# arcee-ai/DALM

Measured on NVIDIA H100. Metric: RAG-e2e train-step samples/sec (bge-large + Llama-2-7B, bs=18), higher is better.
Workload: dtype bf16

## Files before the change

### dalm_b200/_lib.py

```python
from __future__ import annotations

import ctypes
import os
from ctypes import c_char_p, c_float, c_int, c_longlong, c_void_p

_HERE = os.path.dirname(os.path.abspath(__file__))
LIB_PATH = os.path.join(_HERE, "csrc", "libdalm_b200.so")

from ctypes import c_ulonglong

_I, _L, _F, _P, _U = c_int, c_longlong, c_float, c_void_p, c_ulonglong
_DROP = [_F, _U, _U, _P]

SIGNATURES = {
    "dalm_b200_last_error": [],
    "dalm_b200_version": [],
    "dalm_b200_launch_count": [],
    "dalm_b200_reset_launch_count": [],
    "dalm_b200_probe_device": [],
    "dalm_b200_marginal_counts": [_P, _P, _I, _I, _P, _P, _P],
    "dalm_b200_inbatch_loss_fwd_bwd": [_P, _P, _I, _I, _F, _P, _P, _P, _P, _P, _P, _P, _F, _P],
    "dalm_b200_ce_marginal_fwd_bwd": [_P, _P, _I, _P, _P, _P, _P, _I, _I, _I, _L, _F, _P],
    "dalm_b200_ce_marginal_rows": [_P, _P, _I, _P, _P, _P, _P, _I, _I, _I, _L, _F, _I, _I, _P],
    "dalm_b200_finalize_loss": [_P, _P, _I, _I, _P, _P, _P, _P],
    "dalm_b200_bump_counter": [_P, _P],
    "dalm_b200_dropout_scale": [_P, _L, _F, _U, _U, _P, _P],
    "dalm_b200_lora_dx": [_P, _L, _P, _L, _P, _L, _I, _I, _I, _F, _U, _U, _P, _P],
    "dalm_b200_small_matmul_f32": [_P, _P, _P, _I, _I, _I, _I, _I, _F, _P],
    "dalm_b200_gemm_bf16": [_I, _P, _L, _P, _L, _P, _L, _I, _I, _I, _I, _F, _P, _I, _P, _L, _I, _I, _I, *_DROP, _P],
    "dalm_b200_gemm_clear_cache": [],
    "dalm_b200_gemm_set_raster": [_I],
    "dalm_b200_gemm_set_l2_hints": [_I],
    "dalm_b200_attention_fwd": [_P, _L, _P, _L, _P, _L, _P, _P, _L, _P, _I, _I, _I, _I, _I, _F, _I, _I, *_DROP, _P],
    "dalm_b200_attention_tc_fwd": [_P, _L, _P, _L, _P, _L, _P, _P, _L, _P, _I, _I, _I, _I, _I, _F, _I, _I, *_DROP, _P],
    "dalm_b200_attention_tc_bwd": [_P, _L, _P, _L, _P, _L, _P, _P, _L, _P, _P, _L, _P, _P, _L, _P, _L, _P, _L,
                                   _I, _I, _I, _I, _I, _F, _I, _I, *_DROP, _P],
    "dalm_b200_attention_bwd": [_P, _L, _P, _L, _P, _L, _P, _P, _L, _P, _P, _L, _P, _P, _L, _P, _L, _P, _L,
                                _I, _I, _I, _I, _I, _F, _I, _I, *_DROP, _P],
    "dalm_b200_layernorm_fwd": [_P, _P, _P, _P, _P, _L, _P, _P, _I, _I, _F, *_DROP, _P],
    "dalm_b200_layernorm_bwd": [_P, _P, _P, _P, _P, _P, _L, _P, _P, _L, _I, _I, *_DROP, _P],
    "dalm_b200_layernorm_bwd_res": [_P, _P, _P, _P, _P, _P, _L, _P, _P, _P, _L, _I, _I, _P],
    "dalm_b200_rmsnorm_fwd": [_P, _P, _P, _L, _P, _I, _I, _F, _P],
    "dalm_b200_rmsnorm_bwd": [_P, _P, _P, _P, _L, _P, _P, _P, _L, _I, _I, _P],
    "dalm_b200_bert_embed": [_P, _P, _P, _P, _P, _I, _I, _I, _I, _P],
    "dalm_b200_roberta_embed": [_P, _P, _P, _P, _I, _P, _P, _I, _I, _I, _I, _I, _P],
    "dalm_b200_embed_gather": [_P, _P, _P, _I, _I, _I, _P],
    "dalm_b200_rope": [_P, _L, _I, _I, _I, _P, _P, _I, _I, _I, _P],
# ... 40 lines not shown
    "dalm_b200_moe_router_bwd": [_P, _L, _P, _P, _P, _I, _I, _I, _I, _P, _L, _P],
    "dalm_b200_moe_permute": [_P, _I, _I, _I, _P, _P, _P, _P, _P, _P, _P, _P],
    "dalm_b200_moe_gather": [_P, _L, _I, _I, _P, _I, _P, _I, _P, _L, _P],
    "dalm_b200_moe_combine": [_P, _L, _P, _P, _I, _I, _I, _P, _L, _P, _L, _I, _P],
    "dalm_b200_moe_down_bwd": [_P, _L, _P, _L, _P, _P, _I, _I, _P, _P, _L, _P],
}
_RESTYPES = {
    "dalm_b200_last_error": c_char_p,
    "dalm_b200_version": c_char_p,
    "dalm_b200_launch_count": c_longlong,
    "dalm_b200_topk_ip_workspace": c_longlong,
    "dalm_b200_reset_launch_count": None,
    "dalm_b200_gemm_clear_cache": None,
    "dalm_b200_gemm_set_raster": None,
    "dalm_b200_gemm_set_l2_hints": None,
}

_lib = None


class DalmB200Error(RuntimeError):
    pass


def load() -> ctypes.CDLL:
    global _lib
    if _lib is not None:
        return _lib
    if not os.path.exists(LIB_PATH):
        raise DalmB200Error(
# ... 31 lines not shown
```

### dalm_b200/csrc/gemm_wgmma.cu

```cuda
#include "common.cuh"
#include "ptx.cuh"
#include <cudaTypedefs.h>
#include <mutex>
#include <unordered_map>

namespace dalm {
using namespace ptx;

enum class Epi {
  Plain,
  SwiGLU,
  RoPE,
  GeluPair,
  NormRoPE,
};

struct GemmEpilogue {
  void* out;
  long long ldo;
  int out_f32;
  const float* bias;
  const void* resid;
  long long ldr;
  int resid_f32;
// ... 17 lines not shown
__device__ __forceinline__ void tile_coords(int tile, int num_m, int num_n, int gm, int& m_blk, int& n_blk) {
  if (gm <= 0) { m_blk = tile % num_m; n_blk = tile / num_m; return; }
  const int band_tiles = gm * num_n;
  const int band = tile / band_tiles;
  const int r = tile - band * band_tiles;
  const int m0 = band * gm;
  const int h = min(gm, num_m - m0);
  const int n = r / h;
  m_blk = m0 + (r - n * h);
  n_blk = (band & 1) ? (num_n - 1 - n) : n;
}

constexpr int kBoxRows = 64;
constexpr int kBoxBytes = kBoxRows * 128;
constexpr int kStageTileBytes = 2 * kBoxBytes;
constexpr int kEpiGroups = 2;
constexpr int kGemmThreads = 128 + kEpiGroups * 128;

struct EpiStage {
  unsigned char* boxes;
  int bar;
  bool issuer;
  int buf;
  __device__ __forceinline__ unsigned char* begin() {
    if (issuer) bulk_wait_read<1>();
    named_bar_sync(bar, 128);
    return boxes + buf * kBoxBytes;
  }
  __device__ __forceinline__ void end(const CUtensorMap* tm, int col, int row, bool evict_first) {
    fence_proxy_async();
    named_bar_sync(bar, 128);
    if (issuer) {
// ... 267 lines not shown
    }
    sg.end(tmap_out, col0, row0, hint);
    if constexpr (EPI == Epi::GeluPair) {
      box = sg.begin();
#pragma unroll
      for (int i = 0; i < 16; ++i) {
        const float2 p = __bfloat1622float2(pk[i]);
        box_st_bf16x2(box, rb + 8 * (i & 1), 16 * (i >> 1) + 4 * k, gelu_erf(p.x), gelu_erf(p.y));
      }
      sg.end(tmap_out2, col0, row0, false);
    }
    shift8();
  }
}

template <int BN> struct GemmCfg {
  static constexpr int BM = 128, BK = 64;
  static constexpr int A_BYTES = BM * BK * 2;
  static constexpr int B_BYTES = BN * BK * 2;
  static constexpr int STAGE_BYTES = A_BYTES + B_BYTES;
  static constexpr int STAGES = (BN == 256) ? 4 : (BN == 128 ? 6 : 8);
  static constexpr int SMEM_BYTES = STAGES * STAGE_BYTES + kEpiGroups * kStageTileBytes + 1024  + 256 ;
  static_assert(SMEM_BYTES <= 232448, "exceeds 227 KB of shared memory per block");
};

template <int BN, int TA, int TB>
__device__ __forceinline__ void wgmma_tile(float* d, uint64_t da, uint64_t db, int scale_d) {
  if constexpr (BN == 256) wgmma_m64n256k16<TA, TB>(d, da, db, scale_d);
  else if constexpr (BN == 128) wgmma_m64n128k16<TA, TB>(d, da, db, scale_d);
  else wgmma_m64n64k16<TA, TB>(d, da, db, scale_d);
}

template <int BN, int LAYOUT, Epi EPI, int CL, bool GROUPED>
__global__ void __launch_bounds__(kGemmThreads, 1)
gemm_bf16_tn_kernel(const __grid_constant__ CUtensorMap tmap_a, const __grid_constant__ CUtensorMap tmap_b,
                    const __grid_constant__ CUtensorMap tmap_out, const __grid_constant__ CUtensorMap tmap_out2, const GemmEpilogue ep) {
  using Cfg = GemmCfg<BN>;
  constexpr int BM = Cfg::BM, BK = Cfg::BK, STAGES = Cfg::STAGES;
  static_assert(CL == 1 || (LAYOUT == 0 && EPI == Epi::Plain), "the cluster kernel takes the plain TN layout");
  static_assert(!GROUPED || (CL == 1 && LAYOUT <= 1), "the grouped kernel takes the TN and NN layouts on single CTAs");
  extern __shared__ unsigned char smem_raw[];
  unsigned char* smem = reinterpret_cast<unsigned char*>((reinterpret_cast<uintptr_t>(smem_raw) + 1023) & ~uintptr_t(1023));
  unsigned char* staging = smem + STAGES * Cfg::STAGE_BYTES;
  uint64_t* full_bar  = reinterpret_cast<uint64_t*>(staging + kEpiGroups * kStageTileBytes);
  uint64_t* empty_bar = full_bar + STAGES;

  const int warp = threadIdx.x >> 5, lane = threadIdx.x & 31;
  const uint32_t rank = CL == 2 ? cluster_ctarank() : 0u;
  const int M = ep.M, N = ep.N, K = ep.K;
  const int num_m = GROUPED ? min((M + BM - 1) / BM, __ldg(ep.grp_live)) : (M + CL * BM - 1) / (CL * BM);
  const int num_n = (N + BN - 1) / BN;
  const int num_tiles = num_m * num_n;
  const int num_kb = (K + BK - 1) / BK;
  const int unit = blockIdx.x / CL, num_units = gridDim.x / CL;
  const int group_m = CL == 2 ? 0 : ep.group_m;

  if (threadIdx.x == 0) {
    prefetch_tmap(&tmap_a);
    prefetch_tmap(&tmap_b);
    prefetch_tmap(&tmap_out);
    if constexpr (EPI == Epi::SwiGLU || EPI == Epi::GeluPair || EPI == Epi::NormRoPE) prefetch_tmap(&tmap_out2);
  }
  if (threadIdx.x == 32) {
    for (int s = 0; s < STAGES; ++s) { mbar_init(&full_bar[s], 1); mbar_init(&empty_bar[s], 8 * CL); }
    fence_mbar_init();
  }
  if constexpr (CL == 2) cluster_sync_all();
  else __syncthreads();

  if (warp < 4) {
    asm volatile("setmaxnreg.dec.sync.aligned.u32 40;" ::: "memory");
    if (warp == 0 && lane == 0) {
      int stage = 0; uint32_t phase = 0;
      const bool hint_a = (ep.l2_hints & 1) != 0, hint_b = (ep.l2_hints & 2) != 0;
      const uint64_t pol_a = hint_a ? l2_policy_evict_last() : 0ull, pol_b = hint_b ? l2_policy_evict_first() : 0ull;
      auto load = [](void* dst, const CUtensorMap* tm, uint64_t* bar, int c0, int c1, bool hinted, uint64_t pol) {
        if (hinted) tma_load_2d_hint(dst, tm, bar, c0, c1, pol);
        else        tma_load_2d(dst, tm, bar, c0, c1);
      };
      for (int tile = unit; tile < num_tiles; tile += num_units) {
        int m_blk, n_blk;
        tile_coords(tile, num_m, num_n, group_m, m_blk, n_blk);
        const int b_row0 = GROUPED ? __ldg(ep.grp_tiles + m_blk) * (LAYOUT == 1 ? K : N) : 0;
        for (int kb = 0; kb < num_kb; ++kb) {
          mbar_wait(&empty_bar[stage], phase ^ 1);
          unsigned char* sa = smem + stage * Cfg::STAGE_BYTES;
// ... 9 lines not shown
            } else {
              load(sa, &tmap_a, &full_bar[stage], kb * BK, m_blk * BM, hint_a, pol_a);
            }
            if constexpr (LAYOUT >= 1) {
#pragma unroll
              for (int c = 0; c < BN / 64; ++c) load(sb + c * 8192, &tmap_b, &full_bar[stage], n_blk * BN + c * 64, b_row0 + kb * BK, hint_b, pol_b);
            } else {
              load(sb, &tmap_b, &full_bar[stage], kb * BK, b_row0 + n_blk * BN, hint_b, pol_b);
            }
          }
          if (++stage == STAGES) { stage = 0; phase ^= 1; }
        }
      }
    }
  } else {
    asm volatile("setmaxnreg.inc.sync.aligned.u32 232;" ::: "memory");
    const int grp = (warp - 4) >> 2;
    EpiStage sg{staging + grp * kStageTileBytes, 1 + grp, (threadIdx.x & 127) == 0, 0};
    constexpr int TA = LAYOUT == 2 ? 1 : 0, TB = LAYOUT >= 1 ? 1 : 0;
    constexpr uint64_t a_step = TA ? 128 : 2, b_step = TB ? 128 : 2;
    const uint32_t a_off = (uint32_t)grp * 8192u;
    int stage = 0; uint32_t phase = 0;
    for (int tile = unit; tile < num_tiles; tile += num_units) {
      int m_blk, n_blk;
      tile_coords(tile, num_m, num_n, group_m, m_blk, n_blk);
      float acc[BN / 2];
      int prev = -1;
      for (int kb = 0; kb < num_kb; ++kb) {
        mbar_wait(&full_bar[stage], phase);
        const uint32_t sa = smem_u32(smem + stage * Cfg::STAGE_BYTES);
        const uint32_t sb = sa + Cfg::A_BYTES;
        const uint64_t adesc = TA ? make_sw128_mnmajor_desc(sa + a_off, 8192, 1024) : make_sw128_kmajor_desc(sa + a_off);
        const uint64_t bdesc = TB ? make_sw128_mnmajor_desc(sb, 8192, 1024) : make_sw128_kmajor_desc(sb);
        wgmma_fence();
#pragma unroll
        for (int k = 0; k < BK / 16; ++k)
          wgmma_tile<BN, TA, TB>(acc, adesc + a_step * (uint64_t)k, bdesc + b_step * (uint64_t)k, (kb | k) != 0 ? 1 : 0);
        wgmma_commit();
        wgmma_wait<1>();
        if (prev >= 0 && lane == 0) {
          mbar_arrive(&empty_bar[prev]);
          if constexpr (CL == 2) mbar_arrive_remote(&empty_bar[prev], rank ^ 1u);
        }
        prev = stage;
        if (++stage == STAGES) { stage = 0; phase ^= 1; }
      }
      wgmma_wait<0>();
      if (lane == 0) {
        mbar_arrive(&empty_bar[prev]);
        if constexpr (CL == 2) mbar_arrive_remote(&empty_bar[prev], rank ^ 1u);
      }
      epilogue_tile<BN, EPI>(ep, &tmap_out, &tmap_out2, sg, acc, (m_blk * CL + (int)rank) * BM + grp * 64, n_blk * BN);
// ... 51 lines not shown
  CUtensorMap m;
  CUresult r = fn(&m, f32 ? CU_TENSOR_MAP_DATA_TYPE_FLOAT32 : CU_TENSOR_MAP_DATA_TYPE_BFLOAT16, 2, const_cast<void*>(ptr), dims, strides, box, estr,
                  CU_TENSOR_MAP_INTERLEAVE_NONE, CU_TENSOR_MAP_SWIZZLE_128B, CU_TENSOR_MAP_L2_PROMOTION_L2_256B,
                  CU_TENSOR_MAP_FLOAT_OOB_FILL_NONE);
  DALM_REQUIRE(r == CUDA_SUCCESS, "gemm: cuTensorMapEncodeTiled failed (%d) rows=%lld cols=%lld ld=%lld box_rows=%d",
               (int)r, rows, cols, ld, box_rows);
  {
    std::lock_guard<std::mutex> g(g_tmap_mu);
    if (g_tmaps.size() > 8192) g_tmaps.clear();
    g_tmaps[key] = m;
  }
  *out = m;
  return 0;
}

template <int BN, int LAYOUT, Epi EPI, bool GROUPED = false>
static int launch_gemm(const CUtensorMap& ta, const CUtensorMap& tb, const CUtensorMap& to, const GemmEpilogue& ep,
                       int max_ctas, cudaStream_t stream, const CUtensorMap* to2) {
  using Cfg = GemmCfg<BN>;
  static bool attr_set = false;
  if (!attr_set) {
    DALM_CUDA(cudaFuncSetAttribute(gemm_bf16_tn_kernel<BN, LAYOUT, EPI, 1, GROUPED>, cudaFuncAttributeMaxDynamicSharedMemorySize, Cfg::SMEM_BYTES));
    attr_set = true;
  }
  const int num_tiles = ((ep.M + 127) / 128) * ((ep.N + BN - 1) / BN);
  int grid = num_tiles < num_sms() ? num_tiles : num_sms();
  if (max_ctas > 0 && grid > max_ctas) grid = max_ctas;
  gemm_bf16_tn_kernel<BN, LAYOUT, EPI, 1, GROUPED><<<grid, kGemmThreads, Cfg::SMEM_BYTES, stream>>>(ta, tb, to, to2 ? *to2 : to, ep);
  count_launch();
  return check_launch("gemm_bf16_tn_kernel");
}

template <int LAYOUT, Epi EPI, bool GROUPED = false>
static int launch_gemm_bn(int bn, const CUtensorMap& ta, const CUtensorMap& tb, const CUtensorMap& to, const GemmEpilogue& ep,
                          int max_ctas, cudaStream_t stream, const CUtensorMap* to2 = nullptr) {
  if (bn == 256) return launch_gemm<256, LAYOUT, EPI, GROUPED>(ta, tb, to, ep, max_ctas, stream, to2);
  if (bn == 128) return launch_gemm<128, LAYOUT, EPI, GROUPED>(ta, tb, to, ep, max_ctas, stream, to2);
  return launch_gemm<64, LAYOUT, EPI, GROUPED>(ta, tb, to, ep, max_ctas, stream, to2);
}

template <int BN>
static int launch_gemm_cluster(const CUtensorMap& ta, const CUtensorMap& tb, const CUtensorMap& to, const GemmEpilogue& ep,
                               int max_ctas, cudaStream_t stream) {
  using Cfg = GemmCfg<BN>;
  auto kern = gemm_bf16_tn_kernel<BN, 0, Epi::Plain, 2, false>;
  static bool attr_set = false;
  if (!attr_set) {
    DALM_CUDA(cudaFuncSetAttribute(kern, cudaFuncAttributeMaxDynamicSharedMemorySize, Cfg::SMEM_BYTES));
    attr_set = true;
  }
  const int num_tiles = ((ep.M + 255) / 256) * ((ep.N + BN - 1) / BN);
  int clusters = num_tiles < num_sms() / 2 ? num_tiles : num_sms() / 2;
  if (max_ctas > 0 && clusters > max_ctas / 2) clusters = max_ctas / 2 > 0 ? max_ctas / 2 : 1;
  cudaLaunchConfig_t cfg = {};
  cfg.gridDim = dim3(2 * clusters);
  cfg.blockDim = dim3(kGemmThreads);
  cfg.dynamicSmemBytes = Cfg::SMEM_BYTES;
  cfg.stream = stream;
  cudaLaunchAttribute attr[1];
  attr[0].id = cudaLaunchAttributeClusterDimension;
  attr[0].val.clusterDim.x = 2; attr[0].val.clusterDim.y = 1; attr[0].val.clusterDim.z = 1;
  cfg.attrs = attr; cfg.numAttrs = 1;
  DALM_CUDA(cudaLaunchKernelEx(&cfg, kern, ta, tb, to, to, ep));
  count_launch();
  return check_launch("gemm_bf16_tn_kernel (cluster of 2)");
}

}

using namespace dalm;

static int env_int(const char* name, int dflt) {
  const char* v = getenv(name);
  return (v && *v) ? atoi(v) : dflt;
}
static int g_group_m_override = env_int("DALM_B200_GEMM_RASTER", 0);
extern "C" void dalm_b200_gemm_set_raster(int group_m) { g_group_m_override = group_m; }
static int g_l2_hints = env_int("DALM_B200_GEMM_L2_HINTS", -1);
static double l2_resident_a() { return (double)l2_bytes() / 3.0; }
extern "C" void dalm_b200_gemm_set_l2_hints(int mask) { g_l2_hints = mask < 0 ? -1 : (mask & 7); }
static int pick_l2_hints(int M, int N, int K, int tile_n, int group_m, bool stream_out) {
  if (g_l2_hints >= 0) return g_l2_hints;
  const long long tiles = (long long)((M + 127) / 128) * ((N + tile_n - 1) / tile_n);
  return (group_m == 0 && tiles > num_sms() && 2.0 * M * K <= l2_resident_a() && !stream_out) ? 7 : 0;
}

static int pick_block_n(int M, int N) {
  const long long m1 = (M + 127) / 128;
  double best = 1e30;
  int bn = 64;
  const int cand[3] = {256, 128, 64};
  const double penalty[3] = {1.0, 1.55, 2.7};
  for (int i = 0; i < 3; ++i) {
    if (cand[i] > 64 && N < cand[i]) continue;
    const long long tiles = m1 * ((N + cand[i] - 1) / cand[i]);
    const double cost = (double)((tiles + num_sms() - 1) / num_sms()) * cand[i] * penalty[i];
    if (cost < best) { best = cost; bn = cand[i]; }
  }
  return bn;
}

static int pick_group_m(int M, int N, int K, int tile_n, bool stream_out) {
  const int num_m = (M + 127) / 128, num_n = (N + tile_n - 1) / tile_n;
  int group_m = 0;
  if (g_group_m_override > 0) return g_group_m_override;
  if (g_group_m_override == -1 || (long long)num_m * num_n <= num_sms()) return 0;
  const double a_bytes = 2.0 * M * K;
  if (g_group_m_override == 0 && a_bytes <= l2_resident_a() && !stream_out) return 0;
  const double ideal = sqrt((double)num_sms() * tile_n / 128.0);
  int nbands = (int)(num_m / ideal + 0.5);
  if (nbands < 1) nbands = 1;
  group_m = (num_m + nbands - 1) / nbands;
  if (group_m >= num_m) group_m = 0;
  return group_m;
}

static GemmEpilogue gemm_epilogue(int M, int N, int K, int tile_n, void* out, long long ldo, int out_f32 = 0,
                                  const void* resid = nullptr, long long ldr = 0, int resid_f32 = 0) {
  GemmEpilogue ep{};
  ep.out = out; ep.ldo = ldo; ep.out_f32 = out_f32;
  ep.resid = resid; ep.ldr = ldr; ep.resid_f32 = resid_f32;
  ep.alpha = 1.f;
  ep.M = M; ep.N = N; ep.K = K;
  ep.drop = make_drop(0.f, 0, 0, nullptr);
  const bool stream_out = out_f32 != 0 || resid != nullptr;
  ep.group_m = pick_group_m(M, N, K, tile_n, stream_out);
  ep.l2_hints = pick_l2_hints(M, N, K, tile_n, ep.group_m, stream_out);
  return ep;
}

extern "C" int dalm_b200_gemm_bf16(int layout, const void* A, long long lda, const void* B, long long ldb, void* out,
                                   long long ldo, int out_f32, int M, int N, int K, float alpha, const float* bias,
                                   int act, const void* resid, long long ldr, int resid_f32, int block_n,
                                   int max_ctas, float drop_p, unsigned long long drop_seed,
                                   unsigned long long drop_stream_id, const void* drop_offset, void* stream) {
  DALM_REQUIRE(layout >= 0 && layout <= 2, "gemm: layout must be 0 (TN), 1 (NN) or 2 (wgrad)");
  DALM_REQUIRE(M > 0 && N > 0 && K > 0, "gemm: empty problem M=%d N=%d K=%d", M, N, K);
  DALM_REQUIRE((N % 8) == 0, "gemm: N=%d must be a multiple of 8", N);
  DALM_REQUIRE((K % 8) == 0 || layout == 2, "gemm: K=%d must be a multiple of 8", K);
  DALM_REQUIRE((M % 8) == 0 || layout != 2, "gemm: M=%d must be a multiple of 8 for the wgrad layout", M);
  DALM_REQUIRE(lda >= (layout == 2 ? M : K) && ldb >= (layout >= 1 ? N : K) && ldo >= N, "gemm: leading dimensions too small");
  DALM_REQUIRE((ldo % (out_f32 ? 4 : 8)) == 0, "gemm: ldo=%lld breaks 16-byte row alignment", ldo);
  DALM_REQUIRE((reinterpret_cast<uintptr_t>(out) & 15) == 0, "gemm: out is not 16-byte aligned");
  if (resid) {
    DALM_REQUIRE((ldr % (resid_f32 ? 4 : 8)) == 0, "gemm: ldr=%lld breaks 16-byte row alignment", ldr);
    DALM_REQUIRE((reinterpret_cast<uintptr_t>(resid) & 15) == 0, "gemm: resid is not 16-byte aligned");
  }
  DALM_REQUIRE(act == 0 || act == 1 || act == 2, "gemm: act must be 0 (none), 1 (gelu) or 2 (gelu backward: multiply by gelu'(resid))");
  DALM_REQUIRE(act != 2 || (resid != nullptr && !resid_f32 && !out_f32 && drop_p == 0.f),
               "gemm: act 2 (gelu backward) needs a bf16 `resid` (the pre-activation), a bf16 output and no dropout");
  int bn = block_n;
  if (bn == 0) bn = pick_block_n(M, N);
  DALM_REQUIRE(bn == 64 || bn == 128 || bn == 256 || bn == 2128 || bn == 2256,
               "gemm: block_n must be 0, 64/128/256 (single CTA) or 2128/2256 (cluster of two CTAs)");
  const bool pair = bn > 1000;
  DALM_REQUIRE(!(pair && layout != 0), "gemm: the cluster kernel only takes the TN layout");
  const int tile_n = pair ? bn % 1000 : bn;
  CUtensorMap ta, tb, to;
  if (layout == 2) { if (int e = get_tmap(A, K, M, lda, 64, &ta)) return e; }
  else             { if (int e = get_tmap(A, M, K, lda, 128, &ta)) return e; }
  if (layout >= 1) { if (int e = get_tmap(B, K, N, ldb, 64, &tb)) return e; }
  else             { if (int e = get_tmap(B, N, K, ldb, pair ? tile_n / 2 : tile_n, &tb)) return e; }
  if (int e = get_tmap(out, M, N, ldo, kBoxRows, &to, out_f32)) return e;
  DALM_REQUIRE(drop_p >= 0.f && drop_p < 1.f, "gemm: dropout p must be in [0,1)");
  GemmEpilogue ep = gemm_epilogue(M, N, K, tile_n, out, ldo, out_f32, resid, ldr, resid_f32);
  ep.bias = bias; ep.act = act; ep.alpha = alpha;
  ep.drop = make_drop(drop_p, drop_seed, drop_stream_id, drop_offset);
  cudaStream_t st = (cudaStream_t)stream;
  if (bn == 2256) return launch_gemm_cluster<256>(ta, tb, to, ep, max_ctas, st);
  if (bn == 2128) return launch_gemm_cluster<128>(ta, tb, to, ep, max_ctas, st);
  if (layout == 1) return launch_gemm_bn<1, Epi::Plain>(bn, ta, tb, to, ep, max_ctas, st);
  if (layout == 2) return launch_gemm_bn<2, Epi::Plain>(bn, ta, tb, to, ep, max_ctas, st);
  return launch_gemm_bn<0, Epi::Plain>(bn, ta, tb, to, ep, max_ctas, st);
}

extern "C" int dalm_b200_gemm_bf16_swiglu(const void* A, long long lda, const void* B, long long ldb, void* gu, long long ldgu,
                                          void* act, long long ldact, int M, int N, int K, void* stream) {
  DALM_REQUIRE(M > 0 && K > 0 && N >= 256 && (N % 256) == 0, "gemm_swiglu: N=%d must be a positive multiple of 256 (128-feature gate / up blocks)", N);
  DALM_REQUIRE((K % 8) == 0 && lda >= K && ldb >= K && ldgu >= N && ldact >= N / 2, "gemm_swiglu: bad K / leading dimensions");
  DALM_REQUIRE((ldgu % 8) == 0 && (ldact % 8) == 0 && ((uintptr_t)gu & 15) == 0 && ((uintptr_t)act & 15) == 0, "gemm_swiglu: output alignment");
  CUtensorMap ta, tb, to, to2;
  if (int e = get_tmap(A, M, K, lda, 128, &ta)) return e;
  if (int e = get_tmap(B, N, K, ldb, 256, &tb)) return e;
  if (int e = get_tmap(gu, M, N, ldgu, kBoxRows, &to, 0)) return e;
  if (int e = get_tmap(act, M, N / 2, ldact, kBoxRows, &to2, 0)) return e;
  const GemmEpilogue ep = gemm_epilogue(M, N, K, 256, gu, ldgu);
  return launch_gemm<256, 0, Epi::SwiGLU>(ta, tb, to, ep, 0, (cudaStream_t)stream, &to2);
}

extern "C" int dalm_b200_gemm_bf16_gelu(const void* A, long long lda, const void* B, long long ldb, void* pre, long long ldpre,
                                        void* act, long long ldact, int M, int N, int K, const float* bias, void* stream) {
  DALM_REQUIRE(M > 0 && N > 0 && K > 0 && (N % 8) == 0 && (K % 8) == 0, "gemm_gelu: bad shape M=%d N=%d K=%d", M, N, K);
  DALM_REQUIRE(lda >= K && ldb >= K && ldpre >= N && ldact >= N, "gemm_gelu: leading dimensions too small");
  DALM_REQUIRE((ldpre % 8) == 0 && (ldact % 8) == 0 && ((uintptr_t)pre & 15) == 0 && ((uintptr_t)act & 15) == 0, "gemm_gelu: output alignment");
  const int bn = pick_block_n(M, N);
  CUtensorMap ta, tb, to, to2;
  if (int e = get_tmap(A, M, K, lda, 128, &ta)) return e;
  if (int e = get_tmap(B, N, K, ldb, bn, &tb)) return e;
  if (int e = get_tmap(pre, M, N, ldpre, kBoxRows, &to, 0)) return e;
  if (int e = get_tmap(act, M, N, ldact, kBoxRows, &to2, 0)) return e;
  GemmEpilogue ep = gemm_epilogue(M, N, K, bn, pre, ldpre);
  ep.bias = bias;
  return launch_gemm_bn<0, Epi::GeluPair>(bn, ta, tb, to, ep, 0, (cudaStream_t)stream, &to2);
}

extern "C" int dalm_b200_gemm_bf16_rope(const void* A, long long lda, const void* B, long long ldb, void* out, long long ldo, int M,
                                        int N, int K, const float* bias, const float* cos_t, const float* sin_t, int L, int rope_cols,
                                        const float* q_norm, const float* k_norm, int nq_heads, float eps, void* pre_out,
                                        long long ld_pre, float* rstd_out, long long ld_rstd, void* stream) {
  DALM_REQUIRE(M > 0 && N > 0 && K > 0 && (N % 8) == 0 && (K % 8) == 0, "gemm_rope: bad shape M=%d N=%d K=%d", M, N, K);
  DALM_REQUIRE(rope_cols > 0 && rope_cols <= N && (rope_cols % 256) == 0, "gemm_rope: rope_cols=%d must be a multiple of 256 (whole 128-wide heads per tile)", rope_cols);
  DALM_REQUIRE(L > 0 && cos_t != nullptr && sin_t != nullptr && ((uintptr_t)cos_t & 15) == 0 && ((uintptr_t)sin_t & 15) == 0, "gemm_rope: cos / sin tables");
  DALM_REQUIRE(lda >= K && ldb >= K && ldo >= N && (ldo % 8) == 0 && ((uintptr_t)out & 15) == 0, "gemm_rope: leading dimensions / alignment");
  CUtensorMap ta, tb, to;
  if (int e = get_tmap(A, M, K, lda, 128, &ta)) return e;
  if (int e = get_tmap(B, N, K, ldb, 256, &tb)) return e;
  if (int e = get_tmap(out, M, N, ldo, kBoxRows, &to, 0)) return e;
  GemmEpilogue ep = gemm_epilogue(M, N, K, 256, out, ldo);
  ep.bias = bias;
  ep.rope_cos = cos_t; ep.rope_sin = sin_t; ep.rope_L = L; ep.rope_cols = rope_cols;
  if (q_norm == nullptr) {
    DALM_REQUIRE(k_norm == nullptr && pre_out == nullptr && rstd_out == nullptr, "gemm_rope: k_norm / pre_out / rstd_out need q_norm");
    return launch_gemm<256, 0, Epi::RoPE>(ta, tb, to, ep, 0, (cudaStream_t)stream, nullptr);
  }
  DALM_REQUIRE(k_norm != nullptr && nq_heads >= 0 && nq_heads <= rope_cols / 128 && eps >= 0.f, "gemm_rope: norm weights / nq_heads=%d", nq_heads);
  DALM_REQUIRE(rstd_out == nullptr || ld_rstd >= rope_cols / 128, "gemm_rope: ld_rstd=%lld < %d heads", ld_rstd, rope_cols / 128);
  CUtensorMap to2 = to;
  if (pre_out != nullptr) {
    DALM_REQUIRE(ld_pre >= rope_cols && (ld_pre % 8) == 0 && ((uintptr_t)pre_out & 15) == 0, "gemm_rope: pre_out leading dimension / alignment");
    if (int e = get_tmap(pre_out, M, rope_cols, ld_pre, kBoxRows, &to2, 0)) return e;
  }
  ep.q_norm = q_norm; ep.k_norm = k_norm; ep.nq_heads = nq_heads; ep.norm_eps = eps;
  ep.norm_rstd = rstd_out; ep.ld_rstd = ld_rstd; ep.norm_pre = pre_out != nullptr;
  return launch_gemm<256, 0, Epi::NormRoPE>(ta, tb, to, ep, 0, (cudaStream_t)stream, &to2);
}

extern "C" int dalm_b200_gemm_bf16_grouped(int layout, int swiglu, const void* A, long long lda, const void* B, int E, void* out,
                                           long long ldo, void* out2, long long ldo2, int M, int N, int K, const int* tile_expert,
                                           const int* live_tiles, int max_ctas, void* stream) {
  DALM_REQUIRE(layout == 0 || layout == 1, "gemm_grouped: layout must be 0 (TN) or 1 (NN)");
  DALM_REQUIRE(M > 0 && N > 0 && K > 0 && E > 0 && (N % 8) == 0 && (K % 8) == 0, "gemm_grouped: bad shape M=%d N=%d K=%d E=%d", M, N, K, E);
  DALM_REQUIRE(layout == 0 || (K % 64) == 0, "gemm_grouped: the NN layout needs K=%d to be a multiple of 64", K);
  DALM_REQUIRE(!swiglu || (layout == 0 && (N % 256) == 0 && out2 != nullptr && ldo2 >= N / 2 && (ldo2 % 8) == 0 &&
                           ((uintptr_t)out2 & 15) == 0),
               "gemm_grouped: swiglu needs layout 0, N=%d a multiple of 256 and an aligned out2 [M, N/2]", N);
  DALM_REQUIRE(lda >= K && ldo >= N && (ldo % 8) == 0 && ((uintptr_t)out & 15) == 0, "gemm_grouped: leading dimensions / alignment");
  DALM_REQUIRE(tile_expert != nullptr && live_tiles != nullptr, "gemm_grouped: tile_expert and live_tiles are required");
  const int bn = swiglu ? 256 : pick_block_n(M, N);
  CUtensorMap ta, tb, to, to2;
  if (int e = get_tmap(A, M, K, lda, 128, &ta)) return e;
  if (layout == 1) { if (int e = get_tmap(B, (long long)E * K, N, N, 64, &tb)) return e; }
  else             { if (int e = get_tmap(B, (long long)E * N, K, K, bn, &tb)) return e; }
  if (int e = get_tmap(out, M, N, ldo, kBoxRows, &to, 0)) return e;
  GemmEpilogue ep = gemm_epilogue(M, N, K, bn, out, ldo);
  ep.grp_tiles = tile_expert; ep.grp_live = live_tiles;
  cudaStream_t st = (cudaStream_t)stream;
  if (swiglu) {
    if (int e = get_tmap(out2, M, N / 2, ldo2, kBoxRows, &to2, 0)) return e;
    return launch_gemm<256, 0, Epi::SwiGLU, true>(ta, tb, to, ep, max_ctas, st, &to2);
  }
  if (layout == 1) return launch_gemm_bn<1, Epi::Plain, true>(bn, ta, tb, to, ep, max_ctas, st);
  return launch_gemm_bn<0, Epi::Plain, true>(bn, ta, tb, to, ep, max_ctas, st);
}

extern "C" void dalm_b200_gemm_clear_cache() {
  std::lock_guard<std::mutex> g(g_tmap_mu);
  g_tmaps.clear();
}
```

### include/dalm_b200.h

```cpp
#ifndef DALM_B200_H
#define DALM_B200_H
#include <stdint.h>
#ifdef __cplusplus
extern "C" {
#endif

const char* dalm_b200_last_error(void);
const char* dalm_b200_version(void);
long long   dalm_b200_launch_count(void);
void        dalm_b200_reset_launch_count(void);
int         dalm_b200_probe_device(void);

int dalm_b200_marginal_counts(const int64_t* gen_mask, const int64_t* qlen, int B, int L, float* cvec, float* nsum,
                              void* stream);
int dalm_b200_inbatch_loss_fwd_bwd(const float* Q, const float* P, int B, int D, float logit_scale, const float* cvec,
                                   const float* nsum, float* S, float* dlp, float* losses, float* dQ, float* dP,
                                   float grad_out, void* stream);
int dalm_b200_ce_marginal_fwd_bwd(const void* logits, void* dlogits, int dtype, const int64_t* ids, const int64_t* mask,
                                  const float* nsum, float* tok_lp, int B, int L, int V, long long ld, float grad_out,
                                  void* stream);
int dalm_b200_ce_marginal_rows(const void* logits, void* dlogits, int dtype, const int64_t* ids, const int64_t* mask,
                               const float* nsum, float* tok_lp, int B, int L, int V, long long ld, float grad_out,
                               int row0, int nrows, void* stream);
int dalm_b200_finalize_loss(const float* tok_lp, const int64_t* mask, int B, int L, const float* nsum,
// ... 12 lines not shown
int dalm_b200_gemm_bf16(int layout, const void* A, long long lda, const void* B, long long ldb, void* out, long long ldo,
                        int out_f32, int M, int N, int K, float alpha, const float* bias, int act, const void* resid,
                        long long ldr, int resid_f32, int block_n, int max_ctas, float drop_p, unsigned long long drop_seed,
                        unsigned long long drop_stream_id, const void* drop_offset, void* stream);
int dalm_b200_gemm_bf16_swiglu(const void* A, long long lda, const void* B, long long ldb, void* gu, long long ldgu, void* act,
                               long long ldact, int M, int N, int K, void* stream);
int dalm_b200_gemm_bf16_rope(const void* A, long long lda, const void* B, long long ldb, void* out, long long ldo, int M, int N,
                             int K, const float* bias, const float* cos_t, const float* sin_t, int L, int rope_cols,
                             const float* q_norm, const float* k_norm, int nq_heads, float eps, void* pre_out, long long ld_pre,
                             float* rstd_out, long long ld_rstd, void* stream);
int dalm_b200_gemm_bf16_gelu(const void* A, long long lda, const void* B, long long ldb, void* pre, long long ldpre, void* act,
                             long long ldact, int M, int N, int K, const float* bias, void* stream);
void dalm_b200_gemm_clear_cache(void);
void dalm_b200_gemm_set_raster(int group_m);
void dalm_b200_gemm_set_l2_hints(int mask);

int dalm_b200_attention_fwd(const void* q, long long ldq, const void* k, long long ldk, const void* v, long long ldv,
                            const int64_t* mask, void* out, long long ldo, float* lse, int B, int L, int Hq, int Hkv,
                            int D, float scale, int causal, int window, float drop_p, unsigned long long drop_seed,
    unsigned long long drop_stream_id, const void* drop_offset, void* stream);
int dalm_b200_attention_bwd(const void* q, long long ldq, const void* k, long long ldk, const void* v, long long ldv,
                            const int64_t* mask, const void* out, long long ldo, const float* lse, const void* d_out,
                            long long lddo, float* delta, void* dq, long long lddq, void* dk, long long lddk, void* dv,
                            long long lddv, int B, int L, int Hq, int Hkv, int D, float scale, int causal, int window, float drop_p, unsigned long long drop_seed,
    unsigned long long drop_stream_id, const void* drop_offset, void* stream);

int dalm_b200_attention_tc_fwd(const void* q, long long ldq, const void* k, long long ldk, const void* v, long long ldv,
                               const int64_t* mask, void* out, long long ldo, float* lse, int B, int L, int Hq, int Hkv,
                               int D, float scale, int causal, int window, float drop_p, unsigned long long drop_seed,
                               unsigned long long drop_stream_id, const void* drop_offset, void* stream);
// ... 127 lines not shown
```

Before: 74.01.

## Add 192x256 GEMM tiles with three consumer warpgroups for plain TN/NN GEMMs

Adds a 192-row by 256-column tile variant of the warp-specialized wgmma GEMM. It uses three epilogue/consumer warpgroups with rebalanced setmaxnreg budgets, and the stage count is now derived from the shared-memory budget. The tile picker considers the taller tile for plain TN/NN GEMMs through a wave-quantization cost model, controlled by an env flag that defaults to on. The aim is more reuse of each B tile and better wave fill. The trade-offs are fewer pipeline stages and a tighter 160-register limit for consumers, which may cause spills with the split n128 wgmma pair.

```diff
diff --git a/dalm_b200/_lib.py b/dalm_b200/_lib.py
--- a/dalm_b200/_lib.py
+++ b/dalm_b200/_lib.py
@@ -31,6 +31,7 @@
     "dalm_b200_gemm_clear_cache": [],
     "dalm_b200_gemm_set_raster": [_I],
     "dalm_b200_gemm_set_l2_hints": [_I],
+    "dalm_b200_gemm_set_tall_tiles": [_I],
     "dalm_b200_attention_fwd": [_P, _L, _P, _L, _P, _L, _P, _P, _L, _P, _I, _I, _I, _I, _I, _F, _I, _I, *_DROP, _P],
     "dalm_b200_attention_tc_fwd": [_P, _L, _P, _L, _P, _L, _P, _P, _L, _P, _I, _I, _I, _I, _I, _F, _I, _I, *_DROP, _P],
     "dalm_b200_attention_tc_bwd": [_P, _L, _P, _L, _P, _L, _P, _P, _L, _P, _P, _L, _P, _P, _L, _P, _L, _P, _L,
@@ -101,6 +102,7 @@
     "dalm_b200_gemm_clear_cache": None,
     "dalm_b200_gemm_set_raster": None,
     "dalm_b200_gemm_set_l2_hints": None,
+    "dalm_b200_gemm_set_tall_tiles": None,
 }
 
 _lib = None
diff --git a/dalm_b200/csrc/gemm_wgmma.cu b/dalm_b200/csrc/gemm_wgmma.cu
--- a/dalm_b200/csrc/gemm_wgmma.cu
+++ b/dalm_b200/csrc/gemm_wgmma.cu
@@ -55,8 +55,6 @@
 constexpr int kBoxRows = 64;
 constexpr int kBoxBytes = kBoxRows * 128;
 constexpr int kStageTileBytes = 2 * kBoxBytes;
-constexpr int kEpiGroups = 2;
-constexpr int kGemmThreads = 128 + kEpiGroups * 128;
 
 struct EpiStage {
   unsigned char* boxes;
@@ -354,35 +352,46 @@
   }
 }
 
-template <int BN> struct GemmCfg {
-  static constexpr int BM = 128, BK = 64;
+template <int BM_, int BN> struct GemmCfg {
+  static_assert(BM_ == 128 || BM_ == 192, "tiles are 128 or 192 rows");
+  static constexpr int BM = BM_, BK = 64;
+  static constexpr int EPI_GROUPS = BM / 64;
+  static constexpr int THREADS = 128 + EPI_GROUPS * 128;
   static constexpr int A_BYTES = BM * BK * 2;
   static constexpr int B_BYTES = BN * BK * 2;
   static constexpr int STAGE_BYTES = A_BYTES + B_BYTES;
-  static constexpr int STAGES = (BN == 256) ? 4 : (BN == 128 ? 6 : 8);
-  static constexpr int SMEM_BYTES = STAGES * STAGE_BYTES + kEpiGroups * kStageTileBytes + 1024  + 256 ;
+  static constexpr int FIXED_BYTES = EPI_GROUPS * kStageTileBytes + 1024  + 256 ;
+  static constexpr int STAGES = (232448 - FIXED_BYTES) / STAGE_BYTES;
+  static constexpr int SMEM_BYTES = STAGES * STAGE_BYTES + FIXED_BYTES;
   static_assert(SMEM_BYTES <= 232448, "exceeds 227 KB of shared memory per block");
+  static constexpr int PRODUCER_REGS = BM == 128 ? 40 : 32;
+  static constexpr int CONSUMER_REGS = BM == 128 ? 232 : 160;
 };
 
-template <int BN, int TA, int TB>
+template <int BM, int BN, int TA, int TB>
 __device__ __forceinline__ void wgmma_tile(float* d, uint64_t da, uint64_t db, int scale_d) {
-  if constexpr (BN == 256) wgmma_m64n256k16<TA, TB>(d, da, db, scale_d);
+  if constexpr (BN == 256 && BM == 192) {
+    wgmma_m64n128k16<TA, TB>(d, da, db, scale_d);
+    wgmma_m64n128k16<TA, TB>(d + 64, da, db + (16384 >> 4), scale_d);
+  } else if constexpr (BN == 256) wgmma_m64n256k16<TA, TB>(d, da, db, scale_d);
   else if constexpr (BN == 128) wgmma_m64n128k16<TA, TB>(d, da, db, scale_d);
   else wgmma_m64n64k16<TA, TB>(d, da, db, scale_d);
 }
 
-template <int BN, int LAYOUT, Epi EPI, int CL, bool GROUPED>
-__global__ void __launch_bounds__(kGemmThreads, 1)
+template <int BM, int BN, int LAYOUT, Epi EPI, int CL, bool GROUPED>
+__global__ void __launch_bounds__(GemmCfg<BM, BN>::THREADS, 1)
 gemm_bf16_tn_kernel(const __grid_constant__ CUtensorMap tmap_a, const __grid_constant__ CUtensorMap tmap_b,
                     const __grid_constant__ CUtensorMap tmap_out, const __grid_constant__ CUtensorMap tmap_out2, const GemmEpilogue ep) {
-  using Cfg = GemmCfg<BN>;
-  constexpr int BM = Cfg::BM, BK = Cfg::BK, STAGES = Cfg::STAGES;
+  using Cfg = GemmCfg<BM, BN>;
+  constexpr int BK = Cfg::BK, STAGES = Cfg::STAGES;
   static_assert(CL == 1 || (LAYOUT == 0 && EPI == Epi::Plain), "the cluster kernel takes the plain TN layout");
   static_assert(!GROUPED || (CL == 1 && LAYOUT <= 1), "the grouped kernel takes the TN and NN layouts on single CTAs");
+  static_assert(BM == 128 || (CL == 1 && !GROUPED), "the cluster and grouped kernels (MoE segments padded to 128 rows) use 128-row tiles");
+  static_assert(BM == 128 || BN == 256, "192-row tiles are 256 columns wide");
   extern __shared__ unsigned char smem_raw[];
   unsigned char* smem = reinterpret_cast<unsigned char*>((reinterpret_cast<uintptr_t>(smem_raw) + 1023) & ~uintptr_t(1023));
   unsigned char* staging = smem + STAGES * Cfg::STAGE_BYTES;
-  uint64_t* full_bar  = reinterpret_cast<uint64_t*>(staging + kEpiGroups * kStageTileBytes);
+  uint64_t* full_bar  = reinterpret_cast<uint64_t*>(staging + Cfg::EPI_GROUPS * kStageTileBytes);
   uint64_t* empty_bar = full_bar + STAGES;
 
   const int warp = threadIdx.x >> 5, lane = threadIdx.x & 31;
@@ -402,14 +411,14 @@
     if constexpr (EPI == Epi::SwiGLU || EPI == Epi::GeluPair || EPI == Epi::NormRoPE) prefetch_tmap(&tmap_out2);
   }
   if (threadIdx.x == 32) {
-    for (int s = 0; s < STAGES; ++s) { mbar_init(&full_bar[s], 1); mbar_init(&empty_bar[s], 8 * CL); }
+    for (int s = 0; s < STAGES; ++s) { mbar_init(&full_bar[s], 1); mbar_init(&empty_bar[s], 4 * Cfg::EPI_GROUPS * CL); }
     fence_mbar_init();
   }
   if constexpr (CL == 2) cluster_sync_all();
   else __syncthreads();
 
   if (warp < 4) {
-    asm volatile("setmaxnreg.dec.sync.aligned.u32 40;" ::: "memory");
+    asm volatile("setmaxnreg.dec.sync.aligned.u32 %0;" :: "n"(Cfg::PRODUCER_REGS) : "memory");
     if (warp == 0 && lane == 0) {
       int stage = 0; uint32_t phase = 0;
       const bool hint_a = (ep.l2_hints & 1) != 0, hint_b = (ep.l2_hints & 2) != 0;
@@ -449,7 +458,7 @@
       }
     }
   } else {
-    asm volatile("setmaxnreg.inc.sync.aligned.u32 232;" ::: "memory");
+    asm volatile("setmaxnreg.inc.sync.aligned.u32 %0;" :: "n"(Cfg::CONSUMER_REGS) : "memory");
     const int grp = (warp - 4) >> 2;
     EpiStage sg{staging + grp * kStageTileBytes, 1 + grp, (threadIdx.x & 127) == 0, 0};
     constexpr int TA = LAYOUT == 2 ? 1 : 0, TB = LAYOUT >= 1 ? 1 : 0;
@@ -470,7 +479,7 @@
         wgmma_fence();
 #pragma unroll
         for (int k = 0; k < BK / 16; ++k)
-          wgmma_tile<BN, TA, TB>(acc, adesc + a_step * (uint64_t)k, bdesc + b_step * (uint64_t)k, (kb | k) != 0 ? 1 : 0);
+          wgmma_tile<BM, BN, TA, TB>(acc, adesc + a_step * (uint64_t)k, bdesc + b_step * (uint64_t)k, (kb | k) != 0 ? 1 : 0);
         wgmma_commit();
         wgmma_wait<1>();
         if (prev >= 0 && lane == 0) {
@@ -552,19 +561,19 @@
   return 0;
 }
 
-template <int BN, int LAYOUT, Epi EPI, bool GROUPED = false>
+template <int BM, int BN, int LAYOUT, Epi EPI, bool GROUPED = false>
 static int launch_gemm(const CUtensorMap& ta, const CUtensorMap& tb, const CUtensorMap& to, const GemmEpilogue& ep,
                        int max_ctas, cudaStream_t stream, const CUtensorMap* to2) {
-  using Cfg = GemmCfg<BN>;
+  using Cfg = GemmCfg<BM, BN>;
   static bool attr_set = false;
   if (!attr_set) {
-    DALM_CUDA(cudaFuncSetAttribute(gemm_bf16_tn_kernel<BN, LAYOUT, EPI, 1, GROUPED>, cudaFuncAttributeMaxDynamicSharedMemorySize, Cfg::SMEM_BYTES));
+    DALM_CUDA(cudaFuncSetAttribute(gemm_bf16_tn_kernel<BM, BN, LAYOUT, EPI, 1, GROUPED>, cudaFuncAttributeMaxDynamicSharedMemorySize, Cfg::SMEM_BYTES));
     attr_set = true;
   }
-  const int num_tiles = ((ep.M + 127) / 128) * ((ep.N + BN - 1) / BN);
+  const int num_tiles = ((ep.M + BM - 1) / BM) * ((ep.N + BN - 1) / BN);
   int grid = num_tiles < num_sms() ? num_tiles : num_sms();
   if (max_ctas > 0 && grid > max_ctas) grid = max_ctas;
-  gemm_bf16_tn_kernel<BN, LAYOUT, EPI, 1, GROUPED><<<grid, kGemmThreads, Cfg::SMEM_BYTES, stream>>>(ta, tb, to, to2 ? *to2 : to, ep);
+  gemm_bf16_tn_kernel<BM, BN, LAYOUT, EPI, 1, GROUPED><<<grid, Cfg::THREADS, Cfg::SMEM_BYTES, stream>>>(ta, tb, to, to2 ? *to2 : to, ep);
   count_launch();
   return check_launch("gemm_bf16_tn_kernel");
 }
@@ -572,16 +581,16 @@
 template <int LAYOUT, Epi EPI, bool GROUPED = false>
 static int launch_gemm_bn(int bn, const CUtensorMap& ta, const CUtensorMap& tb, const CUtensorMap& to, const GemmEpilogue& ep,
                           int max_ctas, cudaStream_t stream, const CUtensorMap* to2 = nullptr) {
-  if (bn == 256) return launch_gemm<256, LAYOUT, EPI, GROUPED>(ta, tb, to, ep, max_ctas, stream, to2);
-  if (bn == 128) return launch_gemm<128, LAYOUT, EPI, GROUPED>(ta, tb, to, ep, max_ctas, stream, to2);
-  return launch_gemm<64, LAYOUT, EPI, GROUPED>(ta, tb, to, ep, max_ctas, stream, to2);
+  if (bn == 256) return launch_gemm<128, 256, LAYOUT, EPI, GROUPED>(ta, tb, to, ep, max_ctas, stream, to2);
+  if (bn == 128) return launch_gemm<128, 128, LAYOUT, EPI, GROUPED>(ta, tb, to, ep, max_ctas, stream, to2);
+  return launch_gemm<128, 64, LAYOUT, EPI, GROUPED>(ta, tb, to, ep, max_ctas, stream, to2);
 }
 
 template <int BN>
 static int launch_gemm_cluster(const CUtensorMap& ta, const CUtensorMap& tb, const CUtensorMap& to, const GemmEpilogue& ep,
                                int max_ctas, cudaStream_t stream) {
-  using Cfg = GemmCfg<BN>;
-  auto kern = gemm_bf16_tn_kernel<BN, 0, Epi::Plain, 2, false>;
+  using Cfg = GemmCfg<128, BN>;
+  auto kern = gemm_bf16_tn_kernel<128, BN, 0, Epi::Plain, 2, false>;
   static bool attr_set = false;
   if (!attr_set) {
     DALM_CUDA(cudaFuncSetAttribute(kern, cudaFuncAttributeMaxDynamicSharedMemorySize, Cfg::SMEM_BYTES));
@@ -592,7 +601,7 @@
   if (max_ctas > 0 && clusters > max_ctas / 2) clusters = max_ctas / 2 > 0 ? max_ctas / 2 : 1;
   cudaLaunchConfig_t cfg = {};
   cfg.gridDim = dim3(2 * clusters);
-  cfg.blockDim = dim3(kGemmThreads);
+  cfg.blockDim = dim3(Cfg::THREADS);
   cfg.dynamicSmemBytes = Cfg::SMEM_BYTES;
   cfg.stream = stream;
   cudaLaunchAttribute attr[1];
@@ -617,35 +626,42 @@
 static int g_l2_hints = env_int("DALM_B200_GEMM_L2_HINTS", -1);
 static double l2_resident_a() { return (double)l2_bytes() / 3.0; }
 extern "C" void dalm_b200_gemm_set_l2_hints(int mask) { g_l2_hints = mask < 0 ? -1 : (mask & 7); }
-static int pick_l2_hints(int M, int N, int K, int tile_n, int group_m, bool stream_out) {
+static int pick_l2_hints(int M, int N, int K, int tile_m, int tile_n, int group_m, bool stream_out) {
   if (g_l2_hints >= 0) return g_l2_hints;
-  const long long tiles = (long long)((M + 127) / 128) * ((N + tile_n - 1) / tile_n);
+  const long long tiles = (long long)((M + tile_m - 1) / tile_m) * ((N + tile_n - 1) / tile_n);
   return (group_m == 0 && tiles > num_sms() && 2.0 * M * K <= l2_resident_a() && !stream_out) ? 7 : 0;
 }
 
-static int pick_block_n(int M, int N) {
-  const long long m1 = (M + 127) / 128;
+static bool g_tall_tiles = env_int("DALM_B200_GEMM_TALL", 1) != 0;
+extern "C" void dalm_b200_gemm_set_tall_tiles(int on) { g_tall_tiles = on != 0; }
+
+struct GemmTile { int bm, bn; };
+static double tile_cost(int M, int N, int bm, int bn, double penalty) {
+  const long long tiles = (long long)((M + bm - 1) / bm) * ((N + bn - 1) / bn);
+  return (double)((tiles + num_sms() - 1) / num_sms()) * bm * bn * penalty;
+}
+static GemmTile pick_tile(int M, int N, bool tall_ok) {
+  const GemmTile cand[4] = {{128, 256}, {128, 128}, {128, 64}, {192, 256}};
+  const double penalty[4] = {1.0, 1.55, 2.7, 1.0};
+  GemmTile t{128, 64};
   double best = 1e30;
-  int bn = 64;
-  const int cand[3] = {256, 128, 64};
-  const double penalty[3] = {1.0, 1.55, 2.7};
-  for (int i = 0; i < 3; ++i) {
-    if (cand[i] > 64 && N < cand[i]) continue;
-    const long long tiles = m1 * ((N + cand[i] - 1) / cand[i]);
-    const double cost = (double)((tiles + num_sms() - 1) / num_sms()) * cand[i] * penalty[i];
-    if (cost < best) { best = cost; bn = cand[i]; }
-  }
-  return bn;
-}
-
-static int pick_group_m(int M, int N, int K, int tile_n, bool stream_out) {
-  const int num_m = (M + 127) / 128, num_n = (N + tile_n - 1) / tile_n;
+  for (int i = 0; i < (tall_ok && g_tall_tiles ? 4 : 3); ++i) {
+    if (cand[i].bn > 64 && N < cand[i].bn) continue;
+    const double cost = tile_cost(M, N, cand[i].bm, cand[i].bn, penalty[i]);
+    if (cost < best) { best = cost; t = cand[i]; }
+  }
+  return t;
+}
+static int pick_block_n(int M, int N) { return pick_tile(M, N, false).bn; }
+
+static int pick_group_m(int M, int N, int K, int tile_m, int tile_n, bool stream_out) {
+  const int num_m = (M + tile_m - 1) / tile_m, num_n = (N + tile_n - 1) / tile_n;
   int group_m = 0;
   if (g_group_m_override > 0) return g_group_m_override;
   if (g_group_m_override == -1 || (long long)num_m * num_n <= num_sms()) return 0;
   const double a_bytes = 2.0 * M * K;
   if (g_group_m_override == 0 && a_bytes <= l2_resident_a() && !stream_out) return 0;
-  const double ideal = sqrt((double)num_sms() * tile_n / 128.0);
+  const double ideal = sqrt((double)num_sms() * tile_n / tile_m);
   int nbands = (int)(num_m / ideal + 0.5);
   if (nbands < 1) nbands = 1;
   group_m = (num_m + nbands - 1) / nbands;
@@ -653,7 +669,7 @@
   return group_m;
 }
 
-static GemmEpilogue gemm_epilogue(int M, int N, int K, int tile_n, void* out, long long ldo, int out_f32 = 0,
+static GemmEpilogue gemm_epilogue(int M, int N, int K, int tile_m, int tile_n, void* out, long long ldo, int out_f32 = 0,
                                   const void* resid = nullptr, long long ldr = 0, int resid_f32 = 0) {
   GemmEpilogue ep{};
   ep.out = out; ep.ldo = ldo; ep.out_f32 = out_f32;
@@ -662,8 +678,8 @@
   ep.M = M; ep.N = N; ep.K = K;
   ep.drop = make_drop(0.f, 0, 0, nullptr);
   const bool stream_out = out_f32 != 0 || resid != nullptr;
-  ep.group_m = pick_group_m(M, N, K, tile_n, stream_out);
-  ep.l2_hints = pick_l2_hints(M, N, K, tile_n, ep.group_m, stream_out);
+  ep.group_m = pick_group_m(M, N, K, tile_m, tile_n, stream_out);
+  ep.l2_hints = pick_l2_hints(M, N, K, tile_m, tile_n, ep.group_m, stream_out);
   return ep;
 }
 
@@ -688,25 +704,33 @@
   DALM_REQUIRE(act != 2 || (resid != nullptr && !resid_f32 && !out_f32 && drop_p == 0.f),
                "gemm: act 2 (gelu backward) needs a bf16 `resid` (the pre-activation), a bf16 output and no dropout");
   int bn = block_n;
-  if (bn == 0) bn = pick_block_n(M, N);
-  DALM_REQUIRE(bn == 64 || bn == 128 || bn == 256 || bn == 2128 || bn == 2256,
-               "gemm: block_n must be 0, 64/128/256 (single CTA) or 2128/2256 (cluster of two CTAs)");
-  const bool pair = bn > 1000;
+  if (bn == 0) {
+    const GemmTile t = pick_tile(M, N, layout <= 1);
+    bn = t.bm == 192 ? 192256 : t.bn;
+  }
+  DALM_REQUIRE(bn == 64 || bn == 128 || bn == 256 || bn == 192256 || bn == 2128 || bn == 2256,
+               "gemm: block_n must be 0, 64/128/256 or 192256 (single CTA) or 2128/2256 (cluster of two CTAs)");
+  const bool pair = bn == 2128 || bn == 2256, tall = bn == 192256;
   DALM_REQUIRE(!(pair && layout != 0), "gemm: the cluster kernel only takes the TN layout");
-  const int tile_n = pair ? bn % 1000 : bn;
+  DALM_REQUIRE(!(tall && layout == 2), "gemm: 192-row tiles take the TN and NN layouts");
+  const int tile_n = bn % 1000, tile_m = tall ? 192 : 128;
   CUtensorMap ta, tb, to;
   if (layout == 2) { if (int e = get_tmap(A, K, M, lda, 64, &ta)) return e; }
-  else             { if (int e = get_tmap(A, M, K, lda, 128, &ta)) return e; }
+  else             { if (int e = get_tmap(A, M, K, lda, tile_m, &ta)) return e; }
   if (layout >= 1) { if (int e = get_tmap(B, K, N, ldb, 64, &tb)) return e; }
   else             { if (int e = get_tmap(B, N, K, ldb, pair ? tile_n / 2 : tile_n, &tb)) return e; }
   if (int e = get_tmap(out, M, N, ldo, kBoxRows, &to, out_f32)) return e;
   DALM_REQUIRE(drop_p >= 0.f && drop_p < 1.f, "gemm: dropout p must be in [0,1)");
-  GemmEpilogue ep = gemm_epilogue(M, N, K, tile_n, out, ldo, out_f32, resid, ldr, resid_f32);
+  GemmEpilogue ep = gemm_epilogue(M, N, K, tile_m, tile_n, out, ldo, out_f32, resid, ldr, resid_f32);
   ep.bias = bias; ep.act = act; ep.alpha = alpha;
   ep.drop = make_drop(drop_p, drop_seed, drop_stream_id, drop_offset);
   cudaStream_t st = (cudaStream_t)stream;
   if (bn == 2256) return launch_gemm_cluster<256>(ta, tb, to, ep, max_ctas, st);
   if (bn == 2128) return launch_gemm_cluster<128>(ta, tb, to, ep, max_ctas, st);
+  if (tall) {
+    if (layout == 1) return launch_gemm<192, 256, 1, Epi::Plain>(ta, tb, to, ep, max_ctas, st, nullptr);
+    return launch_gemm<192, 256, 0, Epi::Plain>(ta, tb, to, ep, max_ctas, st, nullptr);
+  }
   if (layout == 1) return launch_gemm_bn<1, Epi::Plain>(bn, ta, tb, to, ep, max_ctas, st);
   if (layout == 2) return launch_gemm_bn<2, Epi::Plain>(bn, ta, tb, to, ep, max_ctas, st);
   return launch_gemm_bn<0, Epi::Plain>(bn, ta, tb, to, ep, max_ctas, st);
@@ -722,8 +746,8 @@
   if (int e = get_tmap(B, N, K, ldb, 256, &tb)) return e;
   if (int e = get_tmap(gu, M, N, ldgu, kBoxRows, &to, 0)) return e;
   if (int e = get_tmap(act, M, N / 2, ldact, kBoxRows, &to2, 0)) return e;
-  const GemmEpilogue ep = gemm_epilogue(M, N, K, 256, gu, ldgu);
-  return launch_gemm<256, 0, Epi::SwiGLU>(ta, tb, to, ep, 0, (cudaStream_t)stream, &to2);
+  const GemmEpilogue ep = gemm_epilogue(M, N, K, 128, 256, gu, ldgu);
+  return launch_gemm<128, 256, 0, Epi::SwiGLU>(ta, tb, to, ep, 0, (cudaStream_t)stream, &to2);
 }
 
 extern "C" int dalm_b200_gemm_bf16_gelu(const void* A, long long lda, const void* B, long long ldb, void* pre, long long ldpre,
@@ -737,7 +761,7 @@
   if (int e = get_tmap(B, N, K, ldb, bn, &tb)) return e;
   if (int e = get_tmap(pre, M, N, ldpre, kBoxRows, &to, 0)) return e;
   if (int e = get_tmap(act, M, N, ldact, kBoxRows, &to2, 0)) return e;
-  GemmEpilogue ep = gemm_epilogue(M, N, K, bn, pre, ldpre);
+  GemmEpilogue ep = gemm_epilogue(M, N, K, 128, bn, pre, ldpre);
   ep.bias = bias;
   return launch_gemm_bn<0, Epi::GeluPair>(bn, ta, tb, to, ep, 0, (cudaStream_t)stream, &to2);
 }
@@ -754,12 +778,12 @@
   if (int e = get_tmap(A, M, K, lda, 128, &ta)) return e;
   if (int e = get_tmap(B, N, K, ldb, 256, &tb)) return e;
   if (int e = get_tmap(out, M, N, ldo, kBoxRows, &to, 0)) return e;
-  GemmEpilogue ep = gemm_epilogue(M, N, K, 256, out, ldo);
+  GemmEpilogue ep = gemm_epilogue(M, N, K, 128, 256, out, ldo);
   ep.bias = bias;
   ep.rope_cos = cos_t; ep.rope_sin = sin_t; ep.rope_L = L; ep.rope_cols = rope_cols;
   if (q_norm == nullptr) {
     DALM_REQUIRE(k_norm == nullptr && pre_out == nullptr && rstd_out == nullptr, "gemm_rope: k_norm / pre_out / rstd_out need q_norm");
-    return launch_gemm<256, 0, Epi::RoPE>(ta, tb, to, ep, 0, (cudaStream_t)stream, nullptr);
+    return launch_gemm<128, 256, 0, Epi::RoPE>(ta, tb, to, ep, 0, (cudaStream_t)stream, nullptr);
   }
   DALM_REQUIRE(k_norm != nullptr && nq_heads >= 0 && nq_heads <= rope_cols / 128 && eps >= 0.f, "gemm_rope: norm weights / nq_heads=%d", nq_heads);
   DALM_REQUIRE(rstd_out == nullptr || ld_rstd >= rope_cols / 128, "gemm_rope: ld_rstd=%lld < %d heads", ld_rstd, rope_cols / 128);
@@ -770,7 +794,7 @@
   }
   ep.q_norm = q_norm; ep.k_norm = k_norm; ep.nq_heads = nq_heads; ep.norm_eps = eps;
   ep.norm_rstd = rstd_out; ep.ld_rstd = ld_rstd; ep.norm_pre = pre_out != nullptr;
-  return launch_gemm<256, 0, Epi::NormRoPE>(ta, tb, to, ep, 0, (cudaStream_t)stream, &to2);
+  return launch_gemm<128, 256, 0, Epi::NormRoPE>(ta, tb, to, ep, 0, (cudaStream_t)stream, &to2);
 }
 
 extern "C" int dalm_b200_gemm_bf16_grouped(int layout, int swiglu, const void* A, long long lda, const void* B, int E, void* out,
@@ -790,12 +814,12 @@
   if (layout == 1) { if (int e = get_tmap(B, (long long)E * K, N, N, 64, &tb)) return e; }
   else             { if (int e = get_tmap(B, (long long)E * N, K, K, bn, &tb)) return e; }
   if (int e = get_tmap(out, M, N, ldo, kBoxRows, &to, 0)) return e;
-  GemmEpilogue ep = gemm_epilogue(M, N, K, bn, out, ldo);
+  GemmEpilogue ep = gemm_epilogue(M, N, K, 128, bn, out, ldo);
   ep.grp_tiles = tile_expert; ep.grp_live = live_tiles;
   cudaStream_t st = (cudaStream_t)stream;
   if (swiglu) {
     if (int e = get_tmap(out2, M, N / 2, ldo2, kBoxRows, &to2, 0)) return e;
-    return launch_gemm<256, 0, Epi::SwiGLU, true>(ta, tb, to, ep, max_ctas, st, &to2);
+    return launch_gemm<128, 256, 0, Epi::SwiGLU, true>(ta, tb, to, ep, max_ctas, st, &to2);
   }
   if (layout == 1) return launch_gemm_bn<1, Epi::Plain, true>(bn, ta, tb, to, ep, max_ctas, st);
   return launch_gemm_bn<0, Epi::Plain, true>(bn, ta, tb, to, ep, max_ctas, st);
diff --git a/include/dalm_b200.h b/include/dalm_b200.h
--- a/include/dalm_b200.h
+++ b/include/dalm_b200.h
@@ -50,6 +50,7 @@
 void dalm_b200_gemm_clear_cache(void);
 void dalm_b200_gemm_set_raster(int group_m);
 void dalm_b200_gemm_set_l2_hints(int mask);
+void dalm_b200_gemm_set_tall_tiles(int on);
 
 int dalm_b200_attention_fwd(const void* q, long long ldq, const void* k, long long ldk, const void* v, long long ldv,
                             const int64_t* mask, void* out, long long ldo, float* lse, int B, int L, int Hq, int Hkv,
```

Result: faster. 74.90, median of 6 (+1.2%).
